# revdotcom/reverb

Measured on NVIDIA H100. Metric: rtfx_attention_rescoring_30s_chunks, higher is better.
Workload: dtype bf16

## Files before the change

### include/rvb_b200.h

```cpp
#ifndef RVB_B200_H_
#define RVB_B200_H_

#if defined(__GNUC__)
#define RVB_API __attribute__((visibility("default")))
#else
#define RVB_API
#endif

#ifdef __cplusplus
extern "C" {
#endif

typedef struct rvb_model rvb_model;

typedef struct rvb_model_config {
  int input_dim;
  int d_model;
  int heads;
  int ffn_dim;
  int num_blocks;
  int cnn_kernel;
  int causal;
  int cnn_layer_norm;
  int num_langs;
// ... 19 lines not shown
RVB_API int rvb_model_finalize(rvb_model* m);
RVB_API rvb_model* rvb_model_fork(rvb_model* m);
RVB_API void rvb_model_destroy(rvb_model* m);
RVB_API int rvb_encoder_out_frames(int T);
RVB_API int rvb_encoder_out_len(int feat_len, int T);

RVB_API int rvb_resample(const void* d_wave, int is_i16, long long n_in, const float* d_kernel, int orig, int new_, int width,
                         float* d_out, long long n_out, void* stream);
RVB_API long long rvb_fbank_num_frames(long long n_samples);
RVB_API int rvb_fbank_f32(const float* d_wave, long long n_samples, float* d_feats, long long n_frames, void* stream);
RVB_API int rvb_fbank_i16(const short* d_wave, long long n_samples, float* d_feats, long long n_frames, void* stream);
RVB_API int rvb_fbank_batch(const void* d_wave, int is_i16, int batch, long long wave_stride, long long n_samples,
                            float* d_feats, long long n_frames, void* stream);

RVB_API int rvb_encoder_forward(rvb_model* m, const float* d_feats, const int* h_feat_lens, int B, int T,
                        const float* h_cat_embs, int n_cat, float* d_enc_out, int* h_enc_lens, void* stream);
RVB_API int rvb_encoder_forward_chunked(rvb_model* m, const float* d_feats, const int* h_feat_lens, int B, int T,
                                        const float* h_cat_embs, int n_cat, int chunk_size, int num_left_chunks,
                                        float* d_enc_out, int* h_enc_lens, void* stream);

RVB_API int rvb_encoder_forward_streaming(rvb_model* m, const float* d_feats, int B, int T, const float* h_cat_embs,
                                          int n_cat, int chunk_size, int num_left_chunks, float* d_enc_out,
                                          int* h_enc_lens, void* stream);

RVB_API int rvb_ctc_topk(rvb_model* m, const float* d_enc_out, int B, int Tp, int k, float blank_penalty, int blank_id,
                 float* d_topk_val, int* d_topk_idx, float* d_logp, void* stream);
RVB_API int rvb_logp_topk(const float* d_logp, int rows, int V, int k, float* d_topk_val, int* d_topk_idx, void* stream);

RVB_API int rvb_ctc_greedy_search(const int* d_topk_idx, int k, const int* h_enc_lens, int B, int Tp, int blank_id,
                          int* h_tokens, int* h_lens, void* stream);
RVB_API int rvb_ctc_prefix_beam_search(const float* d_topk_val, const int* d_topk_idx, int k, const int* h_enc_lens, int B,
                               int Tp, int beam, int blank_id, int max_len, int* h_tokens, int* h_times, int* h_lens,
                               double* h_scores, int* h_nhyp, void* stream);

RVB_API int rvb_attention_rescoring(rvb_model* m, const float* d_enc_out, const int* h_enc_lens, int B, int Tp,
                            const int* h_hyp_tokens, const int* h_hyp_lens, int N, int max_len,
                            const float* h_cat_embs, int n_cat, float reverse_weight, float* h_l2r, float* h_r2l,
                            void* stream);

RVB_API int rvb_beam_search_rescoring(rvb_model* m, const float* d_topk_val, const int* d_topk_idx, int k,
                                      const float* d_enc_out, const int* h_enc_lens, int B, int Tp, int beam,
                                      int blank_id, const float* h_cat_embs, int n_cat, float reverse_weight, int cap,
                                      int* h_tokens, int* h_times, int* h_lens, double* h_scores, int* h_nhyp,
                                      float* h_l2r, float* h_r2l, int* out_max_len, void* stream);

RVB_API int rvb_search_submit(rvb_model* m, const float* d_topk_val, const int* d_topk_idx, int k, const float* d_enc_out,
                              const int* h_enc_lens, int B, int Tp, int beam, int blank_id, void* stream);
RVB_API int rvb_rescoring_submit(rvb_model* m, int ticket, const float* h_cat_embs, int n_cat, float reverse_weight, int cap,
                                 int run_decoder, int* h_tokens, int* h_times, float* h_l2r, float* h_r2l,
                                 int* out_max_len, void* stream);
RVB_API int rvb_rescoring_collect(rvb_model* m, int ticket, int* h_lens, double* h_scores, int* h_nhyp);
RVB_API int rvb_ticket_release(rvb_model* m, int ticket);

RVB_API int rvb_decoder_step_topk(rvb_model* m, const float* d_enc_out, const int* h_enc_lens, int B, int Tp, int N,
                                  const int* h_hyps, int L, const float* h_cat_embs, int n_cat, int k, float* h_topk_val,
                                  int* h_topk_idx, void* stream);

RVB_API int rvb_decoder_cache_begin(rvb_model* m, const float* d_enc_out, const int* h_enc_lens, int B, int Tp, int N,
                                    int max_steps, const float* h_cat_embs, int n_cat, void* stream);
RVB_API int rvb_decoder_cache_step(rvb_model* m, const int* h_tokens, const int* h_parents, int k, float* h_topk_val,
                                   int* h_topk_idx, void* stream);
RVB_API int rvb_decoder_cache_end(rvb_model* m);

RVB_API int rvb_decoder_step_logp(rvb_model* m, const float* d_enc_out, const int* h_enc_lens, int B, int Tp, int N,
                                  const int* h_hyps, int L, const float* h_cat_embs, int n_cat, float* h_logp,
                                  void* stream);

RVB_API int rvb_ctc_force_align(const float* d_logp, int V, const int* h_enc_lens, int B, int Tp, const int* h_labels,
                                const int* h_label_lens, int max_U, int blank_id, int* h_frames, int* h_first,
                                int* h_last, int* h_peak, float* h_peak_logp, float* h_score, double* h_loglik,
                                void* stream);

typedef struct rvb_aligner rvb_aligner;
RVB_API long long rvb_aligner_workspace_bytes(int U, int total_frames, int want_loglik);
RVB_API rvb_aligner* rvb_aligner_begin(rvb_model* m, const int* h_labels, int U, int total_frames, int V, int blank_id,
                                       int want_loglik, long long budget_bytes, void* stream);
RVB_API int rvb_aligner_push(rvb_aligner* a, const float* d_logp, int n_rows, void* stream);
RVB_API int rvb_aligner_finish(rvb_aligner* a, int* h_frames, int* h_first, int* h_last, int* h_peak, float* h_peak_logp,
                               float* h_score, double* h_loglik, void* stream);
RVB_API void rvb_aligner_abort(rvb_aligner* a);

RVB_API int rvb_gemm_bf16(const void* d_A, const void* d_W, const float* d_bias, int M, int N, int K, int act, int out_mode,
                  float alpha, void* d_out, int ldo, void* stream);
RVB_API int rvb_gemm_bf16x3(const void* d_A, const void* d_W, const float* d_bias, int M, int N, int K, int act, int out_mode,
                            float alpha, void* d_out, int ldo, void* stream);
RVB_API int rvb_f32_to_bf16_pair(const float* d_x, void* d_out, long long rows, int width, void* stream);
RVB_API long long rvb_gemm_logsoftmax_gather_ws_bytes(int M, int N);
RVB_API int rvb_gemm_logsoftmax_gather(const void* d_A, const void* d_W, const float* d_bias, int M, int N, int K,
                                       const int* d_gather, void* d_ws, float* d_out, void* stream);
RVB_API int rvb_layernorm(const float* d_x, const float* d_gamma, const float* d_beta, float eps, int M, int d,
                  void* d_out_bf16, float* d_out_f32, void* stream);
RVB_API int rvb_attention(const void* d_q, const void* d_k, const void* d_v, const void* d_p, const float* d_bias_u,
                  const float* d_bias_v, void* d_out, int ldq, int ldk, int ldv, int ldp, int ldo, int Bq, int Tq, int Tk,
                  int H, int dk, int q_per_kv, const int* d_k_lens, const int* d_q_lens, int causal, float scale,
                  void* stream);
RVB_API int rvb_attention_tc(const void* d_q, const void* d_k, const void* d_v, void* d_out, int ldq, int ldk, int ldv,
                             int ldo, int groups, int Tq, int Tk, int H, int dk, const float* d_key_bias,
                             const int* d_k_lens, int causal, float scale, void* stream);
RVB_API int rvb_attention_tc_chunked(const void* d_q, const void* d_k, const void* d_v, void* d_out, int ldq, int ldk,
                                     int ldv, int ldo, int groups, int Tq, int Tk, int H, int dk, const float* d_key_bias,
                                     const int* d_k_lens, int chunk, int left_chunks, float scale, void* stream);
RVB_API int rvb_relpos_prep(const void* d_k, int ldk, const void* d_pos, int ldp, const float* d_bias_u,
                            const float* d_bias_v, void* d_kpp, float* d_cbias, int B, int T, int H, int dk,
                            void* stream);
RVB_API int rvb_f32_to_bf16(const float* d_x, void* d_out, long long n, void* stream);

#ifdef __cplusplus
}
#endif
#endif
```

### reverb_b200/_lib.py

```python
from __future__ import annotations

import ctypes as C
import os
from typing import Optional

_HERE = os.path.dirname(os.path.abspath(__file__))
LIB_PATH = os.environ.get("RVB_LIB_PATH") or os.path.join(_HERE, "librvb_b200.so")


class ModelConfig(C.Structure):
    _fields_ = [(n, C.c_int) for n in (
        "input_dim", "d_model", "heads", "ffn_dim", "num_blocks", "cnn_kernel", "causal",
        "cnn_layer_norm", "num_langs", "vocab", "dec_heads", "dec_ffn_dim", "dec_blocks", "r_dec_blocks",
        "sos_id", "eos_id", "precision")]


class SegConfig(C.Structure):
    _fields_ = [(n, C.c_int) for n in (
        "sample_rate", "sinc_filters", "sinc_kernel", "sinc_stride", "conv_channels", "conv_kernel", "lstm_hidden",
        "lstm_layers", "linear_dim", "linear_layers", "num_classes")]


class EmbConfig(C.Structure):
    _fields_ = [("sample_rate", C.c_int), ("num_mel_bins", C.c_int), ("m_channels", C.c_int), ("embed_dim", C.c_int),
                ("blocks", C.c_int * 4)]


_vp, _i, _f, _ll = C.c_void_p, C.c_int, C.c_float, C.c_longlong

SIGNATURES = {
    "rvb_last_error": (C.c_char_p, []),
    "rvb_launch_count": (C.c_ulonglong, []),
    "rvb_set_gemm_impl": (_i, [_i]),
    "rvb_get_gemm_impl": (_i, []),
    "rvb_gemm_profile_begin": (_i, []),
    "rvb_gemm_profile_end": (_i, [_vp, _vp, _vp]),
    "rvb_model_create": (_vp, [C.POINTER(ModelConfig)]),
    "rvb_model_set_tensor": (_i, [_vp, C.c_char_p, _vp, _ll]),
    "rvb_model_finalize": (_i, [_vp]),
    "rvb_model_fork": (_vp, [_vp]),
    "rvb_model_destroy": (None, [_vp]),
    "rvb_encoder_out_frames": (_i, [_i]),
    "rvb_encoder_out_len": (_i, [_i, _i]),
    "rvb_fbank_num_frames": (_ll, [_ll]),
    "rvb_fbank_f32": (_i, [_vp, _ll, _vp, _ll, _vp]),
    "rvb_fbank_i16": (_i, [_vp, _ll, _vp, _ll, _vp]),
    "rvb_fbank_batch": (_i, [_vp, _i, _i, _ll, _ll, _vp, _ll, _vp]),
    "rvb_encoder_forward": (_i, [_vp, _vp, _vp, _i, _i, _vp, _i, _vp, _vp, _vp]),
    "rvb_encoder_forward_chunked": (_i, [_vp, _vp, _vp, _i, _i, _vp, _i, _i, _i, _vp, _vp, _vp]),
    "rvb_encoder_forward_streaming": (_i, [_vp, _vp, _i, _i, _vp, _i, _i, _i, _vp, _vp, _vp]),
    "rvb_ctc_topk": (_i, [_vp, _vp, _i, _i, _i, _f, _i, _vp, _vp, _vp, _vp]),
    "rvb_logp_topk": (_i, [_vp, _i, _i, _i, _vp, _vp, _vp]),
    "rvb_ctc_greedy_search": (_i, [_vp, _i, _vp, _i, _i, _i, _vp, _vp, _vp]),
    "rvb_resample": (_i, [_vp, _i, _ll, _vp, _i, _i, _i, _vp, _ll, _vp]),
    "rvb_ctc_prefix_beam_search": (_i, [_vp, _vp, _i, _vp, _i, _i, _i, _i, _i, _vp, _vp, _vp, _vp, _vp, _vp]),
    "rvb_beam_search_rescoring": (_i, [_vp, _vp, _vp, _i, _vp, _vp, _i, _i, _i, _i, _vp, _i, _f, _i, _vp, _vp, _vp, _vp, _vp,
                                       _vp, _vp, _vp, _vp]),
    "rvb_search_submit": (_i, [_vp, _vp, _vp, _i, _vp, _vp, _i, _i, _i, _i, _vp]),
    "rvb_rescoring_submit": (_i, [_vp, _i, _vp, _i, _f, _i, _i, _vp, _vp, _vp, _vp, _vp, _vp]),
    "rvb_rescoring_collect": (_i, [_vp, _i, _vp, _vp, _vp]),
    "rvb_ticket_release": (_i, [_vp, _i]),
    "rvb_decoder_step_topk": (_i, [_vp, _vp, _vp, _i, _i, _i, _vp, _i, _vp, _i, _i, _vp, _vp, _vp]),
    "rvb_decoder_cache_begin": (_i, [_vp, _vp, _vp, _i, _i, _i, _i, _vp, _i, _vp]),
    "rvb_decoder_cache_step": (_i, [_vp, _vp, _vp, _i, _vp, _vp, _vp]),
    "rvb_decoder_cache_end": (_i, [_vp]),
    "rvb_decoder_step_logp": (_i, [_vp, _vp, _vp, _i, _i, _i, _vp, _i, _vp, _i, _vp, _vp]),
    "rvb_attention_rescoring": (_i, [_vp, _vp, _vp, _i, _i, _vp, _vp, _i, _i, _vp, _i, _f, _vp, _vp, _vp]),
    "rvb_ctc_force_align": (_i, [_vp, _i, _vp, _i, _i, _vp, _vp, _i, _i, _vp, _vp, _vp, _vp, _vp, _vp, _vp, _vp]),
    "rvb_aligner_workspace_bytes": (_ll, [_i, _i, _i]),
    "rvb_aligner_begin": (_vp, [_vp, _vp, _i, _i, _i, _i, _i, _ll, _vp]),
    "rvb_aligner_push": (_i, [_vp, _vp, _i, _vp]),
    "rvb_aligner_finish": (_i, [_vp, _vp, _vp, _vp, _vp, _vp, _vp, _vp, _vp]),
    "rvb_aligner_abort": (None, [_vp]),
    "rvb_gemm_bf16": (_i, [_vp, _vp, _vp, _i, _i, _i, _i, _i, _f, _vp, _i, _vp]),
    "rvb_gemm_bf16x3": (_i, [_vp, _vp, _vp, _i, _i, _i, _i, _i, _f, _vp, _i, _vp]),
    "rvb_f32_to_bf16_pair": (_i, [_vp, _vp, _ll, _i, _vp]),
    "rvb_gemm_logsoftmax_gather_ws_bytes": (_ll, [_i, _i]),
    "rvb_gemm_logsoftmax_gather": (_i, [_vp, _vp, _vp, _i, _i, _i, _vp, _vp, _vp, _vp]),
    "rvb_layernorm": (_i, [_vp, _vp, _vp, _f, _i, _i, _vp, _vp, _vp]),
    "rvb_attention": (_i, [_vp, _vp, _vp, _vp, _vp, _vp, _vp, _i, _i, _i, _i, _i, _i, _i, _i, _i, _i, _i, _vp, _vp,
                           _i, _f, _vp]),
    "rvb_attention_tc_chunked": (_i, [_vp, _vp, _vp, _vp, _i, _i, _i, _i, _i, _i, _i, _i, _i, _vp, _vp, _i, _i, _f, _vp]),
    "rvb_attention_tc": (_i, [_vp, _vp, _vp, _vp, _i, _i, _i, _i, _i, _i, _i, _i, _i, _vp, _vp, _i, _f, _vp]),
    "rvb_relpos_prep": (_i, [_vp, _i, _vp, _i, _vp, _vp, _vp, _vp, _i, _i, _i, _i, _vp]),
    "rvb_f32_to_bf16": (_i, [_vp, _vp, _ll, _vp]),
    "rvb_seg_create": (_vp, [C.POINTER(SegConfig)]),
    "rvb_seg_set_tensor": (_i, [_vp, C.c_char_p, _vp, _ll]),
    "rvb_seg_finalize": (_i, [_vp]),
    "rvb_seg_destroy": (None, [_vp]),
    "rvb_seg_num_frames": (_i, [_vp, _i]),
    "rvb_seg_forward": (_i, [_vp, _vp, _i, _i, _vp, _vp, _vp]),
    "rvb_emb_create": (_vp, [C.POINTER(EmbConfig)]),
    "rvb_emb_set_tensor": (_i, [_vp, C.c_char_p, _vp, _ll]),
    "rvb_emb_finalize": (_i, [_vp]),
    "rvb_emb_destroy": (None, [_vp]),
    "rvb_emb_num_frames": (_i, [_vp, _i]),
    "rvb_emb_forward": (_i, [_vp, _vp, _i, _i, _vp, _i, _i, _vp, _vp, _vp]),
}

_lib: Optional[C.CDLL] = None


def load() -> C.CDLL:
    global _lib
    if _lib is not None:
        return _lib
    if not os.path.exists(LIB_PATH):
        raise RuntimeError(
            f"{LIB_PATH} is missing: build it with `python -m reverb_b200.build` "
            "(or __graft_entry__.build()). reverb_b200 has no CPU fallback.")
    lib = C.CDLL(LIB_PATH)
    for name, (res, args) in SIGNATURES.items():
        if os.environ.get("RVB_LIB_PATH") and not hasattr(lib, name):
            continue
        fn = getattr(lib, name)
        fn.restype = res
        fn.argtypes = args
    _lib = lib
    return lib


def last_error() -> str:
    msg = load().rvb_last_error()
    return msg.decode("utf8", "replace") if msg else ""


def check(rc: int, what: str) -> None:
    if rc != 0:
        raise RuntimeError(f"{what} failed ({rc}): {last_error()}")
```

### reverb_b200/csrc/common.cuh

```cuda
#pragma once
#include <cuda.h>
#include <cuda_bf16.h>
#include <cuda_runtime.h>
#include <stdint.h>
#include <stdio.h>

#include <atomic>

namespace rvb {

void set_error(const char* fmt, ...);
const char* last_error();

#define RVB_CHECK_CUDA(expr)                                                              \
  do {                                                                                    \
    cudaError_t _e = (expr);                                                              \
    if (_e != cudaSuccess) {                                                              \
      rvb::set_error("%s:%d CUDA error %d (%s) in %s", __FILE__, __LINE__, (int)_e,       \
                     cudaGetErrorString(_e), #expr);                                      \
      return -1;                                                                          \
    }                                                                                     \
  } while (0)

#define RVB_REQUIRE(cond, ...)                                                            \
// ... 13 lines not shown

struct DynSmemOptIn {
  static constexpr int kMaxDev = 64;
  std::atomic<size_t> cfg[kMaxDev];
  DynSmemOptIn() {
    for (auto& c : cfg) c.store(0);
  }
  template <typename K>
  int ensure(K kernel, size_t bytes) {
    if (bytes <= 48 * 1024) return 0;
    int dev = 0;
    RVB_CHECK_CUDA(cudaGetDevice(&dev));
    if (dev >= 0 && dev < kMaxDev && cfg[dev].load(std::memory_order_relaxed) >= bytes) return 0;
    RVB_CHECK_CUDA(cudaFuncSetAttribute(kernel, cudaFuncAttributeMaxDynamicSharedMemorySize, (int)bytes));
    if (dev >= 0 && dev < kMaxDev) cfg[dev].store(bytes, std::memory_order_relaxed);
    return 0;
  }
};

__device__ __forceinline__ float2 ffma2(float2 a, float2 b, float2 c) {
  return make_float2(fmaf(a.x, b.x, c.x), fmaf(a.y, b.y, c.y));
}

__device__ __forceinline__ float warp_sum(float v) {
#pragma unroll
  for (int o = 16; o > 0; o >>= 1) v += __shfl_xor_sync(0xffffffffu, v, o);
  return v;
}
__device__ __forceinline__ float warp_max(float v) {
#pragma unroll
  for (int o = 16; o > 0; o >>= 1) v = fmaxf(v, __shfl_xor_sync(0xffffffffu, v, o));
  return v;
}
__device__ __forceinline__ float silu_f(float x) { return x / (1.0f + __expf(-x)); }
__device__ __forceinline__ float sigmoid_f(float x) { return 1.0f / (1.0f + __expf(-x)); }

__device__ __forceinline__ uint32_t pack_bf16x2(float lo, float hi) {
  __nv_bfloat162 t = __floats2bfloat162_rn(lo, hi);
  return *reinterpret_cast<uint32_t*>(&t);
}
__device__ __forceinline__ float2 unpack_bf16x2(uint32_t u) {
  __nv_bfloat162 t = *reinterpret_cast<__nv_bfloat162*>(&u);
  return __bfloat1622float2(t);
}

__device__ __forceinline__ uint32_t smem_u32(const void* p) {
  return static_cast<uint32_t>(__cvta_generic_to_shared(p));
}

__device__ __forceinline__ void mbar_init(uint64_t* bar, uint32_t count) {
  asm volatile("mbarrier.init.shared::cta.b64 [%0], %1;" ::"r"(smem_u32(bar)), "r"(count));
}
__device__ __forceinline__ void fence_barrier_init() {
  asm volatile("fence.mbarrier_init.release.cluster;" ::: "memory");
}
__device__ __forceinline__ void fence_proxy_async() {
  asm volatile("fence.proxy.async.shared::cta;" ::: "memory");
}
__device__ __forceinline__ void mbar_expect_tx(uint64_t* bar, uint32_t bytes) {
  asm volatile("mbarrier.arrive.expect_tx.shared::cta.b64 _, [%0], %1;" ::"r"(smem_u32(bar)), "r"(bytes)
               : "memory");
}
__device__ __forceinline__ void mbar_arrive(uint64_t* bar) {
  asm volatile("mbarrier.arrive.shared::cta.b64 _, [%0];" ::"r"(smem_u32(bar)) : "memory");
}
__device__ __forceinline__ uint32_t mbar_try_wait(uint64_t* bar, uint32_t parity) {
  uint32_t ok;
  asm volatile(
      "{\n"
      ".reg .pred p;\n"
      "mbarrier.try_wait.parity.shared::cta.b64 p, [%1], %2;\n"
      "selp.u32 %0, 1, 0, p;\n"
      "}\n"
      : "=r"(ok)
      : "r"(smem_u32(bar)), "r"(parity)
      : "memory");
  return ok;
}
__device__ __forceinline__ void mbar_wait(uint64_t* bar, uint32_t parity) {
  while (!mbar_try_wait(bar, parity)) {
  }
}

__device__ __forceinline__ void tma_prefetch_desc(const CUtensorMap* m) {
  asm volatile("prefetch.tensormap [%0];" ::"l"(reinterpret_cast<uint64_t>(m)) : "memory");
}
__device__ __forceinline__ void tma_load_4d(void* smem_dst, const CUtensorMap* m, uint64_t* bar, int c0, int c1,
                                            int c2, int c3) {
  asm volatile(
      "cp.async.bulk.tensor.4d.shared::cluster.global.mbarrier::complete_tx::bytes [%0], [%1, {%3, %4, %5, %6}], [%2];"
      ::"r"(smem_u32(smem_dst)),
      "l"(reinterpret_cast<uint64_t>(m)), "r"(smem_u32(bar)), "r"(c0), "r"(c1), "r"(c2), "r"(c3)
      : "memory");
}
__device__ __forceinline__ void tma_load_2d(void* smem_dst, const CUtensorMap* m, uint64_t* bar, int c0, int c1) {
  asm volatile(
      "cp.async.bulk.tensor.2d.shared::cluster.global.mbarrier::complete_tx::bytes [%0], [%1, {%3, %4}], [%2];"
      ::"r"(smem_u32(smem_dst)),
      "l"(reinterpret_cast<uint64_t>(m)), "r"(smem_u32(bar)), "r"(c0), "r"(c1)
      : "memory");
}

__device__ __forceinline__ void wgmma_fence() { asm volatile("wgmma.fence.sync.aligned;" ::: "memory"); }
__device__ __forceinline__ void wgmma_commit() { asm volatile("wgmma.commit_group.sync.aligned;" ::: "memory"); }
template <int N>
__device__ __forceinline__ void wgmma_wait() {
  asm volatile("wgmma.wait_group.sync.aligned %0;" ::"n"(N) : "memory");
}
template <int R>
__device__ __forceinline__ void wgmma_fence_regs(float* d) {
#pragma unroll
  for (int i = 0; i < R; ++i) asm volatile("" : "+f"(d[i])::"memory");
}
__device__ __forceinline__ void wgmma_m64n128k16_ss(float* d, uint64_t adesc, uint64_t bdesc, uint32_t accumulate) {
  asm volatile(
      "{\n"
      ".reg .pred p;\n"
      "setp.ne.b32 p, %66, 0;\n"
      "wgmma.mma_async.sync.aligned.m64n128k16.f32.bf16.bf16 "
      "{%0, %1, %2, %3, %4, %5, %6, %7, %8, %9, %10, %11, %12, %13, %14, %15, %16, %17, %18, %19, %20, %21, %22, %23, %24, %25, %26, %27, %28, %29, %30, %31, %32, %33, %34, %35, %36, %37, %38, %39, %40, %41, %42, %43, %44, %45, %46, %47, %48, %49, %50, %51, %52, %53, %54, %55, %56, %57, %58, %59, %60, %61, %62, %63}, %64, %65, p, 1, 1, 0, 0;\n"
      "}\n"
      : "+f"(d[0]), "+f"(d[1]), "+f"(d[2]), "+f"(d[3]), "+f"(d[4]), "+f"(d[5]), "+f"(d[6]), "+f"(d[7]), "+f"(d[8]), "+f"(d[9]), "+f"(d[10]), "+f"(d[11]), "+f"(d[12]), "+f"(d[13]), "+f"(d[14]), "+f"(d[15]), "+f"(d[16]), "+f"(d[17]), "+f"(d[18]), "+f"(d[19]), "+f"(d[20]), "+f"(d[21]), "+f"(d[22]), "+f"(d[23]), "+f"(d[24]), "+f"(d[25]), "+f"(d[26]), "+f"(d[27]), "+f"(d[28]), "+f"(d[29]), "+f"(d[30]), "+f"(d[31]), "+f"(d[32]), "+f"(d[33]), "+f"(d[34]), "+f"(d[35]), "+f"(d[36]), "+f"(d[37]), "+f"(d[38]), "+f"(d[39]), "+f"(d[40]), "+f"(d[41]), "+f"(d[42]), "+f"(d[43]), "+f"(d[44]), "+f"(d[45]), "+f"(d[46]), "+f"(d[47]), "+f"(d[48]), "+f"(d[49]), "+f"(d[50]), "+f"(d[51]), "+f"(d[52]), "+f"(d[53]), "+f"(d[54]), "+f"(d[55]), "+f"(d[56]), "+f"(d[57]), "+f"(d[58]), "+f"(d[59]), "+f"(d[60]), "+f"(d[61]), "+f"(d[62]), "+f"(d[63])
      : "l"(adesc), "l"(bdesc), "r"(accumulate)
      : "memory");
}
__device__ __forceinline__ void wgmma_m64n64k16_ss(float* d, uint64_t adesc, uint64_t bdesc, uint32_t accumulate) {
  asm volatile(
      "{\n"
      ".reg .pred p;\n"
      "setp.ne.b32 p, %34, 0;\n"
      "wgmma.mma_async.sync.aligned.m64n64k16.f32.bf16.bf16 "
      "{%0, %1, %2, %3, %4, %5, %6, %7, %8, %9, %10, %11, %12, %13, %14, %15, %16, %17, %18, %19, %20, %21, %22, %23, %24, %25, %26, %27, %28, %29, %30, %31}, %32, %33, p, 1, 1, 0, 0;\n"
      "}\n"
      : "+f"(d[0]), "+f"(d[1]), "+f"(d[2]), "+f"(d[3]), "+f"(d[4]), "+f"(d[5]), "+f"(d[6]), "+f"(d[7]), "+f"(d[8]), "+f"(d[9]), "+f"(d[10]), "+f"(d[11]), "+f"(d[12]), "+f"(d[13]), "+f"(d[14]), "+f"(d[15]), "+f"(d[16]), "+f"(d[17]), "+f"(d[18]), "+f"(d[19]), "+f"(d[20]), "+f"(d[21]), "+f"(d[22]), "+f"(d[23]), "+f"(d[24]), "+f"(d[25]), "+f"(d[26]), "+f"(d[27]), "+f"(d[28]), "+f"(d[29]), "+f"(d[30]), "+f"(d[31])
      : "l"(adesc), "l"(bdesc), "r"(accumulate)
      : "memory");
}
__device__ __forceinline__ void wgmma_m64n64k16_rs_tb(float* d, const uint32_t* a, uint64_t bdesc) {
  asm volatile(
      "wgmma.mma_async.sync.aligned.m64n64k16.f32.bf16.bf16 "
      "{%0, %1, %2, %3, %4, %5, %6, %7, %8, %9, %10, %11, %12, %13, %14, %15, %16, %17, %18, %19, %20, %21, %22, %23, %24, %25, %26, %27, %28, %29, %30, %31}, {%32, %33, %34, %35}, %36, 1, 1, 1, 1;\n"
      : "+f"(d[0]), "+f"(d[1]), "+f"(d[2]), "+f"(d[3]), "+f"(d[4]), "+f"(d[5]), "+f"(d[6]), "+f"(d[7]), "+f"(d[8]), "+f"(d[9]), "+f"(d[10]), "+f"(d[11]), "+f"(d[12]), "+f"(d[13]), "+f"(d[14]), "+f"(d[15]), "+f"(d[16]), "+f"(d[17]), "+f"(d[18]), "+f"(d[19]), "+f"(d[20]), "+f"(d[21]), "+f"(d[22]), "+f"(d[23]), "+f"(d[24]), "+f"(d[25]), "+f"(d[26]), "+f"(d[27]), "+f"(d[28]), "+f"(d[29]), "+f"(d[30]), "+f"(d[31])
      : "r"(a[0]), "r"(a[1]), "r"(a[2]), "r"(a[3]), "l"(bdesc)
      : "memory");
}

__device__ __forceinline__ uint64_t make_sw128_desc(uint32_t smem_addr) {
  uint64_t d = 0;
  d |= (uint64_t)((smem_addr >> 4) & 0x3FFF);
  d |= (uint64_t)(1024 >> 4) << 16;
  d |= (uint64_t)(1024 >> 4) << 32;
  d |= (uint64_t)1 << 62;
  return d;
}

__device__ __forceinline__ uint32_t cluster_ctarank() {
  uint32_t r;
  asm volatile("mov.u32 %0, %%cluster_ctarank;" : "=r"(r));
  return r;
}
__device__ __forceinline__ void cluster_sync_all() {
  asm volatile("barrier.cluster.arrive.release.aligned;\n\tbarrier.cluster.wait.acquire.aligned;" ::: "memory");
}

}
```

### reverb_b200/csrc/engine.cu

```cuda
#include <math.h>
#include <stdarg.h>
#include <stdlib.h>
#include <string.h>

#include <atomic>
#include <map>
#include <string>
#include <vector>

#include "../../include/rvb_b200.h"
#include "kernels.h"

namespace rvb {

static thread_local char g_err[1024] = "";
std::atomic<unsigned long long> g_launch_count{0};
void set_error(const char* fmt, ...) {
  va_list ap;
  va_start(ap, fmt);
  vsnprintf(g_err, sizeof(g_err), fmt, ap);
  va_end(ap);
}
const char* last_error() { return g_err; }

// ... 1945 lines not shown
                                      int blank_id, const float* h_cat_embs, int n_cat, float reverse_weight, int cap,
                                      int* h_tokens, int* h_times, int* h_lens, double* h_scores, int* h_nhyp,
                                      float* h_l2r, float* h_r2l, int* out_max_len, void* stream) {
  RVB_REQUIRE(m && d_topk_val && d_topk_idx && d_enc_out && h_enc_lens && h_tokens && h_times && h_lens && h_scores &&
                  h_nhyp && h_l2r && out_max_len && B > 0 && Tp > 0 && cap > 0,
              "rvb_beam_search_rescoring: bad arguments");
  RVB_REQUIRE(m->finalized && m->dec_l.present, "beam_search_rescoring: model has no decoder");
  const int id = rvb_search_submit(m, d_topk_val, d_topk_idx, k, d_enc_out, h_enc_lens, B, Tp, beam, blank_id, stream);
  if (id < 0) return -1;
  if (rvb_rescoring_submit(m, id, h_cat_embs, n_cat, reverse_weight, cap, 1, h_tokens, h_times, h_l2r, h_r2l, out_max_len,
                           stream))
    return -1;
  return rvb_rescoring_collect(m, id, h_lens, h_scores, h_nhyp);
}

RVB_API int rvb_decoder_step_topk(rvb_model* m, const float* d_enc_out, const int* h_enc_lens, int B, int Tp, int N,
                                  const int* h_hyps, int L, const float* h_cat_embs, int n_cat, int k, float* h_topk_val,
                                  int* h_topk_idx, void* stream) {
  RVB_REQUIRE(m && d_enc_out && h_enc_lens && h_hyps && h_topk_val && h_topk_idx && B > 0 && Tp > 0 && N > 0,
              "rvb_decoder_step_topk: bad arguments");
  return rvb::decoder_step_topk(m, d_enc_out, h_enc_lens, B, Tp, N, h_hyps, L, h_cat_embs, n_cat, k, h_topk_val,
                                h_topk_idx, (cudaStream_t)stream);
}

RVB_API int rvb_decoder_cache_begin(rvb_model* m, const float* d_enc_out, const int* h_enc_lens, int B, int Tp, int N,
                                    int max_steps, const float* h_cat_embs, int n_cat, void* stream) {
  RVB_REQUIRE(m && d_enc_out && h_enc_lens, "rvb_decoder_cache_begin: bad arguments");
  return rvb::decoder_cache_begin(m, d_enc_out, h_enc_lens, B, Tp, N, max_steps, h_cat_embs, n_cat, (cudaStream_t)stream);
}

RVB_API int rvb_decoder_cache_step(rvb_model* m, const int* h_tokens, const int* h_parents, int k, float* h_topk_val,
                                   int* h_topk_idx, void* stream) {
  RVB_REQUIRE(m && h_tokens && h_topk_val && h_topk_idx, "rvb_decoder_cache_step: bad arguments");
  return rvb::decoder_cache_step(m, h_tokens, h_parents, k, h_topk_val, h_topk_idx, (cudaStream_t)stream);
}

RVB_API int rvb_decoder_cache_end(rvb_model* m) {
  if (m && m->dcache) {
    m->dcache->release();
    delete m->dcache;
    m->dcache = nullptr;
  }
  return 0;
}

RVB_API int rvb_decoder_step_logp(rvb_model* m, const float* d_enc_out, const int* h_enc_lens, int B, int Tp, int N,
                                  const int* h_hyps, int L, const float* h_cat_embs, int n_cat, float* h_logp,
                                  void* stream) {
  RVB_REQUIRE(m && d_enc_out && h_enc_lens && h_hyps && h_logp && B > 0 && Tp > 0 && N > 0,
              "rvb_decoder_step_logp: bad arguments");
  std::vector<float> val((size_t)B * N);
  std::vector<int> idx((size_t)B * N);
  return rvb::decoder_step_topk(m, d_enc_out, h_enc_lens, B, Tp, N, h_hyps, L, h_cat_embs, n_cat, 1, val.data(), idx.data(),
                                (cudaStream_t)stream, h_logp);
}

RVB_API int rvb_attention_rescoring(rvb_model* m, const float* d_enc_out, const int* h_enc_lens, int B, int Tp,
                            const int* h_hyp_tokens, const int* h_hyp_lens, int N, int max_len,
                            const float* h_cat_embs, int n_cat, float reverse_weight, float* h_l2r, float* h_r2l,
                            void* stream) {
  RVB_REQUIRE(m && d_enc_out && h_enc_lens && h_hyp_tokens && h_hyp_lens && h_l2r && B > 0 && N > 0 && max_len >= 0,
              "rvb_attention_rescoring: bad arguments");
  return rvb::attention_rescoring(m, d_enc_out, h_enc_lens, B, Tp, h_hyp_tokens, h_hyp_lens, N, max_len, h_cat_embs,
                                  n_cat, reverse_weight, h_l2r, h_r2l, (cudaStream_t)stream);
}

RVB_API int rvb_gemm_bf16(const void* d_A, const void* d_W, const float* d_bias, int M, int N, int K, int act, int out_mode,
                  float alpha, void* d_out, int ldo, void* stream) {
  rvb::GemmArgs g;
  g.A = reinterpret_cast<const rvb::bf16*>(d_A);
  g.W = reinterpret_cast<const rvb::bf16*>(d_W);
  g.M = M;
  g.N = N;
  g.K = K;
  g.bias = d_bias;
  g.act = act;
  g.out_mode = out_mode;
  g.alpha = alpha;
  g.out = d_out;
  g.ldo = ldo;
  return rvb::launch_gemm(g, (cudaStream_t)stream);
}

RVB_API int rvb_gemm_bf16x3(const void* d_A, const void* d_W, const float* d_bias, int M, int N, int K, int act, int out_mode,
                            float alpha, void* d_out, int ldo, void* stream) {
  rvb::GemmArgs g;
  g.A = reinterpret_cast<const rvb::bf16*>(d_A);
  g.W = reinterpret_cast<const rvb::bf16*>(d_W);
  g.M = M;
  g.N = N;
  g.K = K;
  g.bias = d_bias;
  g.act = act;
  g.out_mode = out_mode;
  g.alpha = alpha;
  g.out = d_out;
  g.ldo = ldo;
  g.x3 = 1;
  if (out_mode == rvb::OUT_BF16) g.out_split = (act == rvb::ACT_GLU) ? N / 2 : N;
  return rvb::launch_gemm(g, (cudaStream_t)stream);
}

RVB_API int rvb_f32_to_bf16_pair(const float* d_x, void* d_out, long long rows, int width, void* stream) {
  return rvb::launch_f32_to_pair(d_x, reinterpret_cast<rvb::bf16*>(d_out), rows, width, (cudaStream_t)stream);
}

RVB_API long long rvb_gemm_logsoftmax_gather_ws_bytes(int M, int N) {
  return (long long)M * rvb::lse_slabs(N) * (long long)sizeof(float2) + (long long)M * (long long)sizeof(float);
}

RVB_API int rvb_gemm_logsoftmax_gather(const void* d_A, const void* d_W, const float* d_bias, int M, int N, int K,
                                       const int* d_gather, void* d_ws, float* d_out, void* stream) {
  RVB_REQUIRE(d_A && d_W && d_gather && d_ws && d_out, "rvb_gemm_logsoftmax_gather: bad arguments");
  const int slabs = rvb::lse_slabs(N);
  rvb::GemmArgs g;
  g.A = reinterpret_cast<const rvb::bf16*>(d_A);
  g.W = reinterpret_cast<const rvb::bf16*>(d_W);
  g.bias = d_bias;
  g.M = M;
  g.N = N;
  g.K = K;
  g.out_mode = rvb::OUT_LSE;
  g.lse_gather = d_gather;
  g.lse_part = reinterpret_cast<float2*>(d_ws);
  g.lse_tgt = reinterpret_cast<float*>(g.lse_part + (size_t)M * slabs);
  if (rvb::launch_gemm(g, (cudaStream_t)stream)) return -1;
  return rvb::launch_lse_merge(g.lse_part, slabs, g.lse_tgt, d_gather, M, d_out, (cudaStream_t)stream);
}

RVB_API int rvb_layernorm(const float* d_x, const float* d_gamma, const float* d_beta, float eps, int M, int d,
                  void* d_out_bf16, float* d_out_f32, void* stream) {
  return rvb::launch_layernorm(d_x, d_gamma, d_beta, eps, M, d, reinterpret_cast<rvb::bf16*>(d_out_bf16), d_out_f32,
                               nullptr, 0, 0, (cudaStream_t)stream);
}

RVB_API int rvb_attention(const void* d_q, const void* d_k, const void* d_v, const void* d_p, const float* d_bias_u,
                  const float* d_bias_v, void* d_out, int ldq, int ldk, int ldv, int ldp, int ldo, int Bq, int Tq, int Tk,
                  int H, int dk, int q_per_kv, const int* d_k_lens, const int* d_q_lens, int causal, float scale,
                  void* stream) {
  rvb::AttnArgs a;
  a.q = reinterpret_cast<const rvb::bf16*>(d_q);
  a.k = reinterpret_cast<const rvb::bf16*>(d_k);
  a.v = reinterpret_cast<const rvb::bf16*>(d_v);
  a.p = reinterpret_cast<const rvb::bf16*>(d_p);
  a.bias_u = d_bias_u;
  a.bias_v = d_bias_v;
  a.out = reinterpret_cast<rvb::bf16*>(d_out);
  a.ldq = ldq; a.ldk = ldk; a.ldv = ldv; a.ldp = ldp; a.ldo = ldo;
  a.Bq = Bq; a.Tq = Tq; a.Tk = Tk; a.H = H; a.dk = dk;
  a.q_per_kv = q_per_kv;
  a.k_lens = d_k_lens; a.q_lens = d_q_lens;
  a.causal = causal;
  a.scale = scale;
  return rvb::launch_attention(a, (cudaStream_t)stream);
}

RVB_API int rvb_attention_tc(const void* d_q, const void* d_k, const void* d_v, void* d_out, int ldq, int ldk, int ldv,
                             int ldo, int groups, int Tq, int Tk, int H, int dk, const float* d_key_bias,
                             const int* d_k_lens, int causal, float scale, void* stream) {
  rvb::AttnTcArgs a;
  a.q = reinterpret_cast<const rvb::bf16*>(d_q);
  a.k = reinterpret_cast<const rvb::bf16*>(d_k);
  a.v = reinterpret_cast<const rvb::bf16*>(d_v);
  a.out = reinterpret_cast<rvb::bf16*>(d_out);
  a.ldq = ldq; a.ldk = ldk; a.ldv = ldv; a.ldo = ldo;
  a.groups = groups; a.Tq = Tq; a.Tk = Tk; a.H = H; a.dk = dk;
// ... 39 lines not shown
```

### reverb_b200/csrc/gemm.cu

```cuda
#include <cuda.h>
#include <stdlib.h>
#include <string.h>

#include <mutex>
#include <vector>

#include "kernels.h"

namespace rvb {

static int g_gemm_impl = -1;
void set_gemm_impl(int impl) { g_gemm_impl = impl; }
int get_gemm_impl() {
  if (g_gemm_impl < 0) {
    const char* e = getenv("RVB_GEMM");
    g_gemm_impl = (e && strcmp(e, "simt") == 0) ? 1 : (e && strcmp(e, "narrow") == 0) ? 2 : 0;
  }
  return g_gemm_impl;
}

struct GemmKParams {
  int M, N, K, num_k_blocks;
  int tiles_n, num_tiles;
  const float* bias;
// ... 512 lines not shown
  } else if ((EPI == EPI_RESID || EPI == EPI_F32) && p.f32_coalesced) {
    const int slot = lane & 7, rsub = lane >> 3;
    long long ro[8];
#pragma unroll
    for (int it = 0; it < 8; ++it) {
      const long long o = __shfl_sync(0xffffffffu, orow, it * 4 + rsub);
      ro[it] = (o >= 0) ? o * p.ldo + n0_tile + slot * 4 : -1;
    }
    float* out = reinterpret_cast<float*>(p.out);
    float4 r[8];
    if (EPI == EPI_RESID && n0_tile + c0 + slot * 4 + 4 <= p.N) {
#pragma unroll
      for (int it = 0; it < 8; ++it)
        if (ro[it] >= 0) r[it] = *reinterpret_cast<const float4*>(out + ro[it] + c0);
    }
#pragma unroll 1
    for (int c = c0; c < c1; c += 32) {
      if (n0_tile + c >= p.N) break;
      uint32_t acc[32];
      acc_ld32<BN>(accs, arow, c, acc);
      const int n = n0_tile + c + slot * 4;
      const bool vec = (n + 4 <= p.N);
      float4 rn[8];
      const bool pre_next = EPI == EPI_RESID && (c + 32 < c1) && (n + 32 + 4 <= p.N);
      if (pre_next) {
#pragma unroll
        for (int it = 0; it < 8; ++it)
          if (ro[it] >= 0) rn[it] = *reinterpret_cast<const float4*>(out + ro[it] + c + 32);
      }
      float4 b4 = make_float4(0.f, 0.f, 0.f, 0.f);
      if (p.bias != nullptr) {
        if (vec) {
          b4 = __ldg(reinterpret_cast<const float4*>(p.bias + n));
        } else {
          if (n + 0 < p.N) b4.x = __ldg(p.bias + n + 0);
          if (n + 1 < p.N) b4.y = __ldg(p.bias + n + 1);
          if (n + 2 < p.N) b4.z = __ldg(p.bias + n + 2);
        }
      }
#pragma unroll
      for (int j = 0; j < 8; ++j)
        *reinterpret_cast<uint4*>(stage + lane * 32 + ((j ^ (lane & 7)) << 2)) =
            make_uint4(acc[4 * j], acc[4 * j + 1], acc[4 * j + 2], acc[4 * j + 3]);
      __syncwarp();
#pragma unroll
      for (int it = 0; it < 8; ++it) {
        const int row = it * 4 + rsub;
        float4 v = *reinterpret_cast<const float4*>(stage + row * 32 + ((slot ^ (row & 7)) << 2));
        v.x += b4.x; v.y += b4.y; v.z += b4.z; v.w += b4.w;
        if (ro[it] < 0) continue;
        float* o = out + ro[it] + c;
        if (vec) {
          if (EPI == EPI_RESID) {
            r[it].x += p.alpha * v.x; r[it].y += p.alpha * v.y; r[it].z += p.alpha * v.z; r[it].w += p.alpha * v.w;
            *reinterpret_cast<float4*>(o) = r[it];
          } else {
            *reinterpret_cast<float4*>(o) = v;
          }
        } else {
          const float vv[4] = {v.x, v.y, v.z, v.w};
#pragma unroll
          for (int k = 0; k < 3; ++k)
            if (n + k < p.N) o[k] = (EPI == EPI_RESID) ? o[k] + p.alpha * vv[k] : vv[k];
        }
      }
      __syncwarp();
      if (pre_next) {
#pragma unroll
        for (int it = 0; it < 8; ++it) r[it] = rn[it];
      }
    }
  } else {
#pragma unroll 1
    for (int c = c0; c < c1; c += 32) {
      if (n0_tile + c >= p.N) break;
      uint32_t acc[32];
      acc_ld32<BN>(accs, arow, c, acc);
      if (orow >= 0) store_chunk<EPI>(p, orow, n0_tile + c, acc);
    }
  }
}

constexpr int kConsumerWGs = 2;
constexpr int kGemmThreads = 128 * kConsumerWGs + 32;

template <int BN>
struct GemmCfg {
  static constexpr int BM = 128;
  static constexpr int BK = 64;
  static constexpr int STAGES = 4;
  static constexpr uint32_t A_BYTES = BM * BK * 2;
  static constexpr uint32_t B_BYTES = BN * BK * 2;
  static constexpr uint32_t STAGE_BYTES = A_BYTES + B_BYTES;
  static constexpr uint32_t ACC_BYTES = BM * BN * 4;
  static constexpr uint32_t SMEM_BYTES = STAGES * STAGE_BYTES + ACC_BYTES + 8 * 4096  + 256  +
                                         1024 ;
};

template <int BN, int EPI, bool PAIR>
__global__ void __launch_bounds__(kGemmThreads, 1)
gemm_wg_kernel(const __grid_constant__ CUtensorMap tmA, const __grid_constant__ CUtensorMap tmB, const GemmKParams p) {
  using Cfg = GemmCfg<BN>;
  constexpr int STAGES = Cfg::STAGES;
  extern __shared__ uint8_t smem_raw[];
  uint8_t* smem = reinterpret_cast<uint8_t*>((reinterpret_cast<uintptr_t>(smem_raw) + 1023) & ~uintptr_t(1023));
  uint8_t* sA = smem;
  uint8_t* sB = smem + STAGES * Cfg::A_BYTES;
  float* accs = reinterpret_cast<float*>(smem + STAGES * Cfg::STAGE_BYTES);
  float* stage_epi = accs + Cfg::BM * BN;
  uint64_t* bars = reinterpret_cast<uint64_t*>(stage_epi + 8 * 1024);
  uint64_t* full = bars;
  uint64_t* empty = bars + STAGES;

  const int warp = threadIdx.x >> 5;
  const int lane = threadIdx.x & 31;

  if (threadIdx.x == 0) {
    for (int i = 0; i < STAGES; ++i) {
      mbar_init(&full[i], 1);
      mbar_init(&empty[i], 4 * kConsumerWGs);
    }
    fence_barrier_init();
    tma_prefetch_desc(&tmA);
    tma_prefetch_desc(&tmB);
  }
  __syncthreads();
  const int nkb = p.num_k_blocks;

  if (warp == 4 * kConsumerWGs) {
    if (lane == 0) {
      uint32_t stage = 0, phase = 0;
      for (int tile = blockIdx.x; tile < p.num_tiles; tile += gridDim.x) {
        TileCoord t = decode_tile(p, tile, BN);
        for (int kbx = 0; kbx < nkb; ++kbx) {
          const int seg = p.x3 ? kbx / p.kb_seg : 0;
          const int kb = kbx - seg * p.kb_seg;
          const int a_ofs = (seg == 1) ? p.a_lo_ofs : 0, w_ofs = (seg == 2) ? p.w_lo_ofs : 0;
          mbar_wait(&empty[stage], phase ^ 1);
          mbar_expect_tx(&full[stage], Cfg::STAGE_BYTES);
          if (p.conv_mode) {
            int tap = kb / p.conv_cblocks;
            int cb = kb - tap * p.conv_cblocks;
            int kh = tap / 3, kw = tap - kh * 3;
            tma_load_4d(sA + stage * Cfg::A_BYTES, &tmA, &full[stage], cb * 64 + a_ofs, 2 * t.f + kw, t.row0 + (kh >> 1),
                        t.b * 2 + (kh & 1));
          } else {
            tma_load_4d(sA + stage * Cfg::A_BYTES, &tmA, &full[stage], kb * 64 + a_ofs, t.row0, 0, 0);
          }
          tma_load_2d(sB + stage * Cfg::B_BYTES, &tmB, &full[stage], kb * 64 + w_ofs, t.n0);
          if (++stage == STAGES) {
            stage = 0;
            phase ^= 1;
          }
        }
      }
    }
  } else {
    const int wg = warp >> 2, wl = warp & 3;
    const int q = 2 * wg + (wl & 1);
    const int chalf = wl >> 1;
    constexpr bool whole = (EPI == EPI_LSE || EPI == EPI_GLU || BN == 64);
    const int c0 = whole ? (chalf ? BN : 0) : chalf * (BN / 2);
    const int c1 = whole ? BN : c0 + BN / 2;
    float* stage_w = stage_epi + warp * 1024;
    uint32_t stage = 0, phase = 0;
    float acc[BN / 2];
    for (int tile = blockIdx.x; tile < p.num_tiles; tile += gridDim.x) {
      TileCoord t = decode_tile(p, tile, BN);
#pragma unroll
      for (int i = 0; i < BN / 2; ++i) acc[i] = 0.f;
      int prev = -1;
      for (int kb = 0; kb < nkb; ++kb) {
        mbar_wait(&full[stage], phase);
        const uint64_t adesc = make_sw128_desc(smem_u32(sA + stage * Cfg::A_BYTES + wg * (Cfg::A_BYTES / 2)));
        const uint64_t bdesc = make_sw128_desc(smem_u32(sB + stage * Cfg::B_BYTES));
        wgmma_fence_regs<BN / 2>(acc);
        wgmma_fence();
#pragma unroll
        for (int k = 0; k < 4; ++k) {
          if constexpr (BN == 128) wgmma_m64n128k16_ss(acc, adesc + 2 * k, bdesc + 2 * k, 1u);
          else wgmma_m64n64k16_ss(acc, adesc + 2 * k, bdesc + 2 * k, 1u);
        }
        wgmma_commit();
        wgmma_wait<1>();
        wgmma_fence_regs<BN / 2>(acc);
        if (prev >= 0 && lane == 0) mbar_arrive(&empty[prev]);
        prev = (int)stage;
        if (++stage == STAGES) {
          stage = 0;
          phase ^= 1;
        }
      }
      wgmma_wait<0>();
      wgmma_fence_regs<BN / 2>(acc);
      if (prev >= 0 && lane == 0) mbar_arrive(&empty[prev]);
      asm volatile("bar.sync %0, 128;" ::"r"(1 + wg) : "memory");
      {
        const int r0 = wg * 64 + wl * 16 + (lane >> 2);
#pragma unroll
        for (int j = 0; j < BN / 8; ++j) {
          const int c = 8 * j + 2 * (lane & 3);
#pragma unroll
          for (int i = 0; i < 2; ++i) {
            const int r = r0 + 8 * i;
            *reinterpret_cast<float2*>(accs + r * BN + ((((c >> 2)) ^ (r & 7)) << 2) + (c & 3)) =
                make_float2(acc[4 * j + 2 * i], acc[4 * j + 2 * i + 1]);
          }
        }
      }
      asm volatile("bar.sync %0, 128;" ::"r"(1 + wg) : "memory");
      drain_tile<BN, EPI, PAIR>(p, t, q, lane, accs, c0, c1, stage_w);
    }
  }
}

__device__ __forceinline__ float load_a_elem(const GemmKParams& p, const TileCoord& t, int r, int k) {
  if (k >= p.K) return 0.0f;
  if (p.conv_mode) {
    int tp = t.row0 + r;
    if (tp >= p.conv_T2) return 0.0f;
    int tap = k / p.conv_C;
    int c = k - tap * p.conv_C;
    int kh = tap / 3, kw = tap - kh * 3;
    long long idx = (((long long)(t.b * 2 + (kh & 1)) * p.conv_T1h + (tp + (kh >> 1))) * p.conv_F1 + (2 * t.f + kw)) *
                        p.conv_C + c;
    return __bfloat162float(p.A[idx]);
  }
  int m = t.row0 + r;
  if (m >= p.M) return 0.0f;
  return __bfloat162float(p.A[(long long)m * p.lda + k]);
}

__global__ void __launch_bounds__(256) gemm_simt_kernel(const GemmKParams p) {
  __shared__ float sA[128][17];
  __shared__ float sW[32][17];
  __shared__ float sG[32][17];
  const bool glu = (p.act == ACT_GLU);
  for (int tile = blockIdx.x; tile < p.num_tiles; tile += gridDim.x) {
    TileCoord t = decode_tile(p, tile, 32);
    const int tx = threadIdx.x & 7, ty = threadIdx.x >> 3;
    const int wrow0 = glu ? 2 * t.n0 : t.n0;
    float acc[4][4], accg[4][4];
#pragma unroll
    for (int i = 0; i < 4; ++i)
#pragma unroll
      for (int j = 0; j < 4; ++j) acc[i][j] = accg[i][j] = 0.f;
    for (int k0 = 0; k0 < p.K; k0 += 16) {
      for (int e = threadIdx.x; e < 128 * 16; e += 256) {
        int r = e >> 4, kk = e & 15;
        sA[r][kk] = load_a_elem(p, t, r, k0 + kk);
      }
      for (int e = threadIdx.x; e < 32 * 16; e += 256) {
        int n = e >> 4, kk = e & 15;
        int gn = wrow0 + n, gk = k0 + kk;
        sW[n][kk] = (gn < p.N && gk < p.K) ? __bfloat162float(p.W[(long long)gn * p.ldw + gk]) : 0.f;
        sG[n][kk] = (glu && gn + 32 < p.N && gk < p.K) ? __bfloat162float(p.W[(long long)(gn + 32) * p.ldw + gk]) : 0.f;
      }
      __syncthreads();
#pragma unroll
      for (int kk = 0; kk < 16; ++kk) {
        float a[4], w[4], g[4];
#pragma unroll
        for (int i = 0; i < 4; ++i) a[i] = sA[ty * 4 + i][kk];
#pragma unroll
        for (int j = 0; j < 4; ++j) {
          w[j] = sW[tx * 4 + j][kk];
          g[j] = sG[tx * 4 + j][kk];
        }
#pragma unroll
        for (int i = 0; i < 4; ++i)
#pragma unroll
          for (int j = 0; j < 4; ++j) {
            acc[i][j] = fmaf(a[i], w[j], acc[i][j]);
            accg[i][j] = fmaf(a[i], g[j], accg[i][j]);
          }
      }
      __syncthreads();
    }
    for (int i = 0; i < 4; ++i) {
      long long orow = output_row(p, t, ty * 4 + i);
      if (orow < 0) continue;
      for (int j = 0; j < 4; ++j) {
        int n = t.n0 + tx * 4 + j;
        if (glu) {
          if (2 * n >= p.N) continue;
          const int wr = wrow0 + tx * 4 + j;
          float va = acc[i][j], vg = accg[i][j];
          if (p.bias) {
            va += p.bias[wr];
            vg += p.bias[wr + 32];
          }
          reinterpret_cast<bf16*>(p.out)[orow * p.ldo + n] = __float2bfloat16(va / (1.f + expf(-vg)));
          continue;
        }
// ... 273 lines not shown
```

Baseline: 11110.

## Use ping-pong consumer warpgroups with register reallocation in persistent GEMM

Switches the GEMM from two cooperative consumer warpgroups that split each tile into a ping-pong scheme. Each warpgroup now owns a whole 128-row tile and the two alternate tiles, handing off through new turn and accfree mbarriers, so one group's epilogue can overlap the other's MMA mainloop. A full producer warpgroup is added that uses setmaxnreg to give its registers to the consumers, which now hold twice the accumulators. The change also adds a rows-limited GEMM API entry point. In exchange, the epilogue staging buffer is shared and reduced, and the extra barrier handoffs make correctness harder to verify.

Result: faster. 11920, median of 6 (+7.3%).

```diff
diff --git a/include/rvb_b200.h b/include/rvb_b200.h
--- a/include/rvb_b200.h
+++ b/include/rvb_b200.h
@@ -125,6 +125,9 @@
 
 RVB_API int rvb_gemm_bf16(const void* d_A, const void* d_W, const float* d_bias, int M, int N, int K, int act, int out_mode,
                   float alpha, void* d_out, int ldo, void* stream);
+RVB_API int rvb_gemm_bf16_rows(const void* d_A, const void* d_W, const float* d_bias, int M, int N, int K, int act,
+                               int out_mode, float alpha, void* d_out, int ldo, const int* d_row_lens, int rows_per_batch,
+                               void* stream);
 RVB_API int rvb_gemm_bf16x3(const void* d_A, const void* d_W, const float* d_bias, int M, int N, int K, int act, int out_mode,
                             float alpha, void* d_out, int ldo, void* stream);
 RVB_API int rvb_f32_to_bf16_pair(const float* d_x, void* d_out, long long rows, int width, void* stream);
diff --git a/reverb_b200/_lib.py b/reverb_b200/_lib.py
--- a/reverb_b200/_lib.py
+++ b/reverb_b200/_lib.py
@@ -73,6 +73,7 @@
     "rvb_aligner_finish": (_i, [_vp, _vp, _vp, _vp, _vp, _vp, _vp, _vp, _vp]),
     "rvb_aligner_abort": (None, [_vp]),
     "rvb_gemm_bf16": (_i, [_vp, _vp, _vp, _i, _i, _i, _i, _i, _f, _vp, _i, _vp]),
+    "rvb_gemm_bf16_rows": (_i, [_vp, _vp, _vp, _i, _i, _i, _i, _i, _f, _vp, _i, _vp, _i, _vp]),
     "rvb_gemm_bf16x3": (_i, [_vp, _vp, _vp, _i, _i, _i, _i, _i, _f, _vp, _i, _vp]),
     "rvb_f32_to_bf16_pair": (_i, [_vp, _vp, _ll, _i, _vp]),
     "rvb_gemm_logsoftmax_gather_ws_bytes": (_ll, [_i, _i]),
diff --git a/reverb_b200/csrc/common.cuh b/reverb_b200/csrc/common.cuh
--- a/reverb_b200/csrc/common.cuh
+++ b/reverb_b200/csrc/common.cuh
@@ -119,6 +119,15 @@
   }
 }
 
+template <uint32_t N>
+__device__ __forceinline__ void setmaxnreg_dec() {
+  asm volatile("setmaxnreg.dec.sync.aligned.u32 %0;" ::"n"(N));
+}
+template <uint32_t N>
+__device__ __forceinline__ void setmaxnreg_inc() {
+  asm volatile("setmaxnreg.inc.sync.aligned.u32 %0;" ::"n"(N));
+}
+
 __device__ __forceinline__ void tma_prefetch_desc(const CUtensorMap* m) {
   asm volatile("prefetch.tensormap [%0];" ::"l"(reinterpret_cast<uint64_t>(m)) : "memory");
 }
diff --git a/reverb_b200/csrc/engine.cu b/reverb_b200/csrc/engine.cu
--- a/reverb_b200/csrc/engine.cu
+++ b/reverb_b200/csrc/engine.cu
@@ -2051,6 +2051,26 @@
   return rvb::launch_gemm(g, (cudaStream_t)stream);
 }
 
+RVB_API int rvb_gemm_bf16_rows(const void* d_A, const void* d_W, const float* d_bias, int M, int N, int K, int act,
+                               int out_mode, float alpha, void* d_out, int ldo, const int* d_row_lens, int rows_per_batch,
+                               void* stream) {
+  rvb::GemmArgs g;
+  g.A = reinterpret_cast<const rvb::bf16*>(d_A);
+  g.W = reinterpret_cast<const rvb::bf16*>(d_W);
+  g.M = M;
+  g.N = N;
+  g.K = K;
+  g.bias = d_bias;
+  g.act = act;
+  g.out_mode = out_mode;
+  g.alpha = alpha;
+  g.out = d_out;
+  g.ldo = ldo;
+  g.row_lens = d_row_lens;
+  g.rows_per_batch = rows_per_batch;
+  return rvb::launch_gemm(g, (cudaStream_t)stream);
+}
+
 RVB_API int rvb_gemm_bf16x3(const void* d_A, const void* d_W, const float* d_bias, int M, int N, int K, int act, int out_mode,
                             float alpha, void* d_out, int ldo, void* stream) {
   rvb::GemmArgs g;
diff --git a/reverb_b200/csrc/gemm.cu b/reverb_b200/csrc/gemm.cu
--- a/reverb_b200/csrc/gemm.cu
+++ b/reverb_b200/csrc/gemm.cu
@@ -618,7 +618,9 @@
 }
 
 constexpr int kConsumerWGs = 2;
-constexpr int kGemmThreads = 128 * kConsumerWGs + 32;
+constexpr int kGemmThreads = 128 * (1 + kConsumerWGs);
+constexpr int kProducerRegs = 40;
+constexpr int kConsumerRegs = 232;
 
 template <int BN>
 struct GemmCfg {
@@ -629,8 +631,8 @@
   static constexpr uint32_t B_BYTES = BN * BK * 2;
   static constexpr uint32_t STAGE_BYTES = A_BYTES + B_BYTES;
   static constexpr uint32_t ACC_BYTES = BM * BN * 4;
-  static constexpr uint32_t SMEM_BYTES = STAGES * STAGE_BYTES + ACC_BYTES + 8 * 4096  + 256  +
-                                         1024 ;
+  static constexpr uint32_t SMEM_BYTES = STAGES * STAGE_BYTES + ACC_BYTES + 4 * 4096  +
+                                         256  + 1024 ;
 };
 
 template <int BN, int EPI, bool PAIR>
@@ -644,9 +646,11 @@
   uint8_t* sB = smem + STAGES * Cfg::A_BYTES;
   float* accs = reinterpret_cast<float*>(smem + STAGES * Cfg::STAGE_BYTES);
   float* stage_epi = accs + Cfg::BM * BN;
-  uint64_t* bars = reinterpret_cast<uint64_t*>(stage_epi + 8 * 1024);
+  uint64_t* bars = reinterpret_cast<uint64_t*>(stage_epi + 4 * 1024);
   uint64_t* full = bars;
   uint64_t* empty = bars + STAGES;
+  uint64_t* turn = bars + 2 * STAGES;
+  uint64_t* accfree = turn + 2;
 
   const int warp = threadIdx.x >> 5;
   const int lane = threadIdx.x & 31;
@@ -654,7 +658,11 @@
   if (threadIdx.x == 0) {
     for (int i = 0; i < STAGES; ++i) {
       mbar_init(&full[i], 1);
-      mbar_init(&empty[i], 4 * kConsumerWGs);
+      mbar_init(&empty[i], 4);
+    }
+    for (int w = 0; w < kConsumerWGs; ++w) {
+      mbar_init(&turn[w], 128);
+      mbar_init(&accfree[w], 128);
     }
     fence_barrier_init();
     tma_prefetch_desc(&tmA);
@@ -663,8 +671,9 @@
   __syncthreads();
   const int nkb = p.num_k_blocks;
 
-  if (warp == 4 * kConsumerWGs) {
-    if (lane == 0) {
+  if (warp < 4) {
+    setmaxnreg_dec<kProducerRegs>();
+    if (warp == 0 && lane == 0) {
       uint32_t stage = 0, phase = 0;
       for (int tile = blockIdx.x; tile < p.num_tiles; tile += gridDim.x) {
         TileCoord t = decode_tile(p, tile, BN);
@@ -692,34 +701,40 @@
       }
     }
   } else {
-    const int wg = warp >> 2, wl = warp & 3;
-    const int q = 2 * wg + (wl & 1);
-    const int chalf = wl >> 1;
-    constexpr bool whole = (EPI == EPI_LSE || EPI == EPI_GLU || BN == 64);
-    const int c0 = whole ? (chalf ? BN : 0) : chalf * (BN / 2);
-    const int c1 = whole ? BN : c0 + BN / 2;
-    float* stage_w = stage_epi + warp * 1024;
-    uint32_t stage = 0, phase = 0;
-    float acc[BN / 2];
-    for (int tile = blockIdx.x; tile < p.num_tiles; tile += gridDim.x) {
+    setmaxnreg_inc<kConsumerRegs>();
+    const int wg = (warp >> 2) - 1, wl = warp & 3;
+    float* stage_w = stage_epi + wl * 1024;
+    float acc[BN];
+    for (int i = wg; blockIdx.x + i * gridDim.x < p.num_tiles; i += kConsumerWGs) {
+      const int tile = blockIdx.x + i * gridDim.x;
       TileCoord t = decode_tile(p, tile, BN);
-#pragma unroll
-      for (int i = 0; i < BN / 2; ++i) acc[i] = 0.f;
+      const uint32_t u0 = (uint32_t)i * (uint32_t)nkb;
+      uint32_t stage = u0 % STAGES, phase = (u0 / STAGES) & 1;
+      const uint32_t hand_parity = ((i - 1) >> 1) & 1;
+#pragma unroll
+      for (int e = 0; e < BN; ++e) acc[e] = 0.f;
+      if (i > 0) mbar_wait(&turn[wg], hand_parity);
       int prev = -1;
       for (int kb = 0; kb < nkb; ++kb) {
         mbar_wait(&full[stage], phase);
-        const uint64_t adesc = make_sw128_desc(smem_u32(sA + stage * Cfg::A_BYTES + wg * (Cfg::A_BYTES / 2)));
+        const uint64_t adesc = make_sw128_desc(smem_u32(sA + stage * Cfg::A_BYTES));
         const uint64_t bdesc = make_sw128_desc(smem_u32(sB + stage * Cfg::B_BYTES));
-        wgmma_fence_regs<BN / 2>(acc);
+        constexpr uint64_t kHalfA = (Cfg::A_BYTES / 2) >> 4;
+        wgmma_fence_regs<BN>(acc);
         wgmma_fence();
 #pragma unroll
         for (int k = 0; k < 4; ++k) {
-          if constexpr (BN == 128) wgmma_m64n128k16_ss(acc, adesc + 2 * k, bdesc + 2 * k, 1u);
-          else wgmma_m64n64k16_ss(acc, adesc + 2 * k, bdesc + 2 * k, 1u);
+          if constexpr (BN == 128) {
+            wgmma_m64n128k16_ss(acc, adesc + 2 * k, bdesc + 2 * k, 1u);
+            wgmma_m64n128k16_ss(acc + BN / 2, adesc + kHalfA + 2 * k, bdesc + 2 * k, 1u);
+          } else {
+            wgmma_m64n64k16_ss(acc, adesc + 2 * k, bdesc + 2 * k, 1u);
+            wgmma_m64n64k16_ss(acc + BN / 2, adesc + kHalfA + 2 * k, bdesc + 2 * k, 1u);
+          }
         }
         wgmma_commit();
         wgmma_wait<1>();
-        wgmma_fence_regs<BN / 2>(acc);
+        wgmma_fence_regs<BN>(acc);
         if (prev >= 0 && lane == 0) mbar_arrive(&empty[prev]);
         prev = (int)stage;
         if (++stage == STAGES) {
@@ -727,25 +742,28 @@
           phase ^= 1;
         }
       }
+      mbar_arrive(&turn[wg ^ 1]);
       wgmma_wait<0>();
-      wgmma_fence_regs<BN / 2>(acc);
+      wgmma_fence_regs<BN>(acc);
       if (prev >= 0 && lane == 0) mbar_arrive(&empty[prev]);
-      asm volatile("bar.sync %0, 128;" ::"r"(1 + wg) : "memory");
-      {
-        const int r0 = wg * 64 + wl * 16 + (lane >> 2);
+      if (i > 0) mbar_wait(&accfree[wg], hand_parity);
+#pragma unroll
+      for (int h = 0; h < 2; ++h) {
+        const int r0 = h * 64 + wl * 16 + (lane >> 2);
 #pragma unroll
         for (int j = 0; j < BN / 8; ++j) {
           const int c = 8 * j + 2 * (lane & 3);
 #pragma unroll
-          for (int i = 0; i < 2; ++i) {
-            const int r = r0 + 8 * i;
+          for (int e = 0; e < 2; ++e) {
+            const int r = r0 + 8 * e;
             *reinterpret_cast<float2*>(accs + r * BN + ((((c >> 2)) ^ (r & 7)) << 2) + (c & 3)) =
-                make_float2(acc[4 * j + 2 * i], acc[4 * j + 2 * i + 1]);
+                make_float2(acc[h * (BN / 2) + 4 * j + 2 * e], acc[h * (BN / 2) + 4 * j + 2 * e + 1]);
           }
         }
       }
       asm volatile("bar.sync %0, 128;" ::"r"(1 + wg) : "memory");
-      drain_tile<BN, EPI, PAIR>(p, t, q, lane, accs, c0, c1, stage_w);
+      drain_tile<BN, EPI, PAIR>(p, t, wl, lane, accs, 0, BN, stage_w);
+      mbar_arrive(&accfree[wg ^ 1]);
     }
   }
 }
```
